# robin-karlsson0/pc-accumulation-lib

Measured on AMD Instinct MI355X. Metric: Mpoints/s projected+accumulated and BEV frames/s @256x256; 1/2/4/8 GPU, higher is better.
Workload: dtype f64; 1 GPU; KITTI-360 single forward cam, 120k pts/frame, 200 m horizon (~201 live frames, 5169634 stored pts), one 256x256x21 BEV per integrated frame; points_per_frame=120000, bev_px=256, view_m=80

## Files before the change

pc-accumulation-lib_amd/csrc/pca_bev.hip:

```cpp
#include "pca_bev_common.h"
#include "pca_k1_body.h"
#include <cstdlib>
#include <mutex>

#define KEY_INVALID 0xffffffffu
#define TS 8
#define TCELLS (TS * TS)
#define NFK (2 * TCELLS)
#ifndef AB_THREADS
#define AB_THREADS 1024
#endif
#define MAX_G 512
#ifndef BIN_RUNR
#define BIN_RUNR 4
#endif
#ifndef BIN_WPE
#define BIN_WPE 4
#endif
#ifndef BIN_UNR
#define BIN_UNR 4
#endif
#ifndef BIN_REG_P
#define BIN_REG_P 12
#endif
#ifndef C_THREADS
#define C_THREADS 256
#endif
#define C_WAVES (C_THREADS / 64)
#define C_HIST_WAVES 4
#define RGB_CAP 4096
#ifndef C_SLOT_Q
#define C_SLOT_Q 4
#endif
#define CONTIG_MIN 2560
#define HEAVY_MIN_DEFAULT 2560
#define FLAG_ROAD (1u << 24)
#define FLAG_DYNOBJ (1u << 25)

struct __attribute__((aligned(16))) RecF { double z; uint32_t iw; uint32_t cw; };
struct RecD { double z; double inten; uint32_t c; uint32_t fk; };

struct alignas(16) BevArgs {
    pca_store st;
    const double *intensity64;
    const int64_t *frame_off;
    int slot_begin, slot_split, slot_end;
    int64_t max_points;
    pca_bev_params prm;
    int n_pend;
    int write_back;
    int pend_slot_end[PCA_BEV_MAX_CHAIN];
    Mat34 pend_T[PCA_BEV_MAX_CHAIN];
    int tx, T, G;
    int Gr, Gp;
    int tile_mult;
    int heavy_min;
    int stagger;
    uint32_t *key;
    uint32_t *bh;
    uint32_t *boff;
    int Gk;
    int bin_first, bin_end;
    int k1_slot, k1_n;
    uint32_t *bh0;
    int split;
    uint32_t *heavy_hint;
    uint32_t heavy_hint_known;
    uint32_t *span_hint;
    uint32_t span_hint_known;
    int heavy_launched;
    uint32_t *heavy;
    void *recs;
    double *planes;
    uint16_t *planes_f16;
    double *extra;
    uint32_t *status;
    int dbg;
    int band_r0, band_rows;
};
#define HQ_CLASSES 32
#define HQ_CURSOR 32
#define HQ_DONE 33
#define HQ_IDS 64

struct Window { int64_t lo, hi, sp, c_lo, c_hi; };

__device__ __forceinline__ int chunk_index(const BevArgs &a, int64_t lo, int64_t sp, int64_t chunk)
{
    (void)a; (void)lo; (void)sp; (void)chunk;
    return (int)blockIdx.x;
}
#define K1_SEG 4096
#define K1_RIDE 32
__device__ __forceinline__ int64_t window_end(const BevArgs &a)
{
    const int e = a.Gk ? a.k1_slot : a.slot_end;
    return a.frame_off[a.bin_end < e ? a.bin_end : e];
}
__device__ __forceinline__ int64_t window_begin(const BevArgs &a) { return a.frame_off[a.bin_first]; }
__device__ __forceinline__ Window chunk_of(const BevArgs &a, int &g)
{
    Window w;
    w.lo = window_begin(a);
    const int64_t hi0 = window_end(a);
    w.sp = (a.Gk && a.slot_split > a.k1_slot) ? hi0 : a.frame_off[a.slot_split];
    w.hi = (hi0 - w.lo > a.max_points) ? w.lo + a.max_points : hi0;
    const int G = a.G - a.Gk;
    const int64_t chunk = (w.hi - w.lo + G - 1) / G;
    g = chunk_index(a, w.lo, w.sp, chunk);
    const int c = g - a.Gk;
    w.c_lo = w.lo + (int64_t)c * chunk;
    w.c_hi = w.c_lo + chunk < w.hi ? w.c_lo + chunk : w.hi;
    if (w.c_lo > w.hi) w.c_lo = w.c_hi = w.hi;
    return w;
}
__host__ __device__ __forceinline__ int64_t seg_stride(int64_t n, int G) { return (n + G - 1) / G; }
__device__ __forceinline__ bool bev_split(const BevArgs &a, int64_t window_points)
{
    return a.split == 2 || (a.split == 1 && window_points <= (int64_t)(a.G - a.Gk) * BIN_REG_P * AB_THREADS);
}
__device__ __forceinline__ int table_pos(const BevArgs &a, int g) { return a.Gp ? (g & 7) * a.Gp + (g >> 3) : g; }
__device__ __forceinline__ int table_group(const BevArgs &a, int p)
{
    if (!a.Gp) return p;
    const int x = p / a.Gp;
    return (p - x * a.Gp) * 8 + x;
}

struct BinPoint { double x, y, z; uint32_t key; };
struct PendHi { int64_t v[PCA_BEV_MAX_CHAIN]; };
__device__ __forceinline__ bool apply_owed(const BevArgs &a, const PendHi &pend_hi, int64_t p, double &X, double &Y, double &Z)
{
    bool moved = false;
#pragma unroll 1
    for (int k = 0; k < a.n_pend; ++k) {
        const int64_t hi = k == 0 ? pend_hi.v[0] : k == 1 ? pend_hi.v[1] : k == 2 ? pend_hi.v[2] : pend_hi.v[3];
        if (p < hi) {
            const Mat34 &T = a.pend_T[k];
            const double nx = row4(T.m + 0, X, Y, Z), ny = row4(T.m + 4, X, Y, Z), nz = row4(T.m + 8, X, Y, Z);
            X = nx; Y = ny; Z = nz;
            moved = true;
        }
    }
    return moved;
}
__device__ __forceinline__ uint32_t view_key(const BevArgs &a, const Window &w, int64_t p, double X, double Y, double Z, uint8_t D)
{
    const pca_bev_params &q = a.prm;
    const double v = q.view, vlo = -0.5 * v, vhi = 0.5 * v, pxd = (double)q.px, half_px = 0.5 * pxd;
    const bool use_h = !(q.height_filter != q.height_filter);
    const double x = X - q.origin[0];
    const double y = Y - q.origin[1];
    const double z = Z - q.origin[2];
    double ax = q.R[0] * x; ax = fma(q.R[1], y, ax); ax = fma(q.R[2], z, ax);
    double ay = q.R[3] * x; ay = fma(q.R[4], y, ay); ay = fma(q.R[5], z, ay);
    double az = q.R[6] * x; az = fma(q.R[7], y, az); az = fma(q.R[8], z, az);
    ax += q.dx;
    ay += q.dy;
    bool keep = (ax > vlo) && (ax < vhi) && (ay > vlo) && (ay < vhi);
    if (use_h) keep = keep && (az < q.height_filter);
    keep = keep && (D != 1);
    uint32_t key = KEY_INVALID;
    if (keep) {
        int i = (int)floor(ax / v * pxd + half_px);
        int j = (int)floor(ay / v * pxd + half_px);
        i = i > q.px - 1 ? q.px - 1 : (i < 0 ? 0 : i);
        j = j > q.px - 1 ? q.px - 1 : (j < 0 ? 0 : j);
        const int row = q.px - 1 - j, col = i;
        const uint32_t tile = (uint32_t)((row / TS) * a.tx + (col / TS));
        const uint32_t fk = (uint32_t)(((row % TS) * TS + (col % TS)) * 2) + (p >= w.sp ? 1u : 0u);
        key = (tile << 7) | fk;
    }
    return key;
}
struct ViewConst;
template <bool BAND = false>
__device__ __forceinline__ uint32_t view_key_lean(const ViewConst &c, double X, double Y, double Z, bool live, uint32_t set);
template <bool BAND>
__device__ __forceinline__ BinPoint bin_point(const BevArgs &a, const ViewConst &vc, const Window &w, const PendHi &pend_hi, int64_t p,
                                              double X, double Y, double Z, uint8_t D)
{
    BinPoint r;
    const bool moved = apply_owed(a, pend_hi, p, X, Y, Z);
    if (moved && a.write_back) { a.st.x[p] = X; a.st.y[p] = Y; a.st.z[p] = Z; }
    r.x = X; r.y = Y; r.z = Z;
    r.key = view_key_lean<BAND>(vc, X, Y, Z, D != 1, p >= w.sp ? 1u : 0u);
    return r;
}
template <bool I64>
__device__ __forceinline__ void bin_store(const BevArgs &a, const uint32_t *dynbits, uint32_t pos, uint32_t key, uint32_t rgbs, double z_store,
                                          double iv, float iv32)
{
    const pca_bev_params &q = a.prm;
    const unsigned sem = rgbs >> 24;
    uint32_t c = rgbs & 0xffffffu;
    if ((int)sem == q.road_class) c |= FLAG_ROAD;
    if ((dynbits[sem >> 5] >> (sem & 31u)) & 1u) c |= FLAG_DYNOBJ;
    const double z = z_store - q.origin[2];
    if (I64) {
        RecD r; r.z = z; r.inten = iv; r.c = c; r.fk = key & 127u;
        reinterpret_cast<RecD *>(a.recs)[pos] = r;
    } else {
        const float fi = iv32;
        if (fi < 0.0f) pca_raise(a.status, PCA_STATUS_NEGATIVE_INTENSITY);
        RecF r; r.z = z;
        r.iw = (__float_as_uint(fi) & 0x7fffffffu) | ((key & 1u) << 31);
        r.cw = c | (((key & 127u) >> 1) << 26);
        reinterpret_cast<RecF *>(a.recs)[pos] = r;
    }
}

struct ViewConst { double ox, oy, oz, r0, r1, r3, r4, dx, dy, vlo, vhi, v, rv, pxd, half_px, hf; int px, tx; bool use_h; uint32_t br0, brows; };
__device__ __forceinline__ ViewConst view_const(const BevArgs &a)
{
    const pca_bev_params &q = a.prm;
    ViewConst c;
    c.ox = q.origin[0]; c.oy = q.origin[1]; c.oz = q.origin[2];
    c.r0 = q.R[0]; c.r1 = q.R[1]; c.r3 = q.R[3]; c.r4 = q.R[4];
    c.dx = q.dx; c.dy = q.dy;
    c.v = q.view; c.rv = 1.0 / q.view; c.vlo = -0.5 * q.view; c.vhi = 0.5 * q.view; c.pxd = (double)q.px; c.half_px = 0.5 * c.pxd;
    c.hf = q.height_filter; c.use_h = !(q.height_filter != q.height_filter);
    c.px = q.px; c.tx = a.tx;
    c.br0 = (uint32_t)a.band_r0; c.brows = (uint32_t)a.band_rows;
    return c;
}
template <bool BAND>
__device__ __forceinline__ uint32_t view_key_lean(const ViewConst &c, double X, double Y, double Z, bool live, uint32_t set)
{
    const double x = X - c.ox, y = Y - c.oy;
    const double ax = fma(c.r1, y, c.r0 * x) + c.dx;
    const double ay = fma(c.r4, y, c.r3 * x) + c.dy;
    bool keep = live && (ax > c.vlo) && (ax < c.vhi) && (ay > c.vlo) && (ay < c.vhi) && (fabs(Z) < __builtin_huge_val());
    if (c.use_h) keep = keep && (Z - c.oz < c.hf);
    uint32_t key = KEY_INVALID;
    if (keep) {
// ... 583 lines not shown
}
__device__ __forceinline__ void hist16_add(uint32_t *row, unsigned val, uint32_t times)
{
    atomicAdd(&row[val >> 1], times << (16 * (val & 1)));
}
__device__ __forceinline__ void hist16_medians(TileStats &S, const uint32_t *row_p, const uint32_t *row_f, int cell, int ch,
                                               uint32_t n_p, uint32_t n_f)
{
    const uint4 p = hist16_bins(row_p), f = hist16_bins(row_f);
    const uint4 u = make_uint4(p.x + f.x, p.y + f.y, p.z + f.z, p.w + f.w);
    const uint32_t s_p = p.x + p.y + p.z + p.w, s_f = f.x + f.y + f.z + f.w;
    const uint32_t e_p = wave_incl_scan_add(s_p) - s_p, e_f = wave_incl_scan_add(s_f) - s_f;
    const uint32_t m_p = hist_med2_scanned(p, e_p, s_p, n_p), m_f = hist_med2_scanned(f, e_f, s_f, n_f),
                   m_u = hist_med2_scanned(u, e_p + e_f, s_p + s_f, n_p + n_f);
    if ((threadIdx.x & 63) == 0) { S.med2[0][cell][ch] = m_p; S.med2[1][cell][ch] = m_f; S.med2[2][cell][ch] = m_u; }
}

struct TileLds {
    TileStats S;
    uint32_t off[NFK + 1];
    uint32_t n_big;
    union {
        unsigned long long bits[TCELLS][24];
        uint32_t whist[C_HIST_WAVES][2][3][128];
        uint16_t owner[RGB_CAP];
    };
};

__device__ __forceinline__ void small_cells_bitplanes(TileLds &L, const uint32_t *s_rgb)
{
    const int lane = threadIdx.x & 63, wave = threadIdx.x >> 6;
    constexpr int PER_WAVE = TCELLS / C_WAVES;
    static_assert(PER_WAVE <= 64, "one lane per cell of the wave");
    uint32_t n_mine = 0;
    if (lane < PER_WAVE) n_mine = L.S.cnt[2 * (C_WAVES * lane + wave)] + L.S.cnt[2 * (C_WAVES * lane + wave) + 1];
    unsigned long long half = __ballot(n_mine >= 1 && n_mine <= 32), full = __ballot(n_mine > 32 && n_mine <= 64);
    while (half) {
        const int ia = __ffsll(half) - 1;
        half &= half - 1;
        const int ib = half ? __ffsll(half) - 1 : -1;
        half &= half - 1;
        const int i = lane < 32 ? ia : ib;
        const int l = lane & 31;
        uint32_t v = 0;
        int cell = 0;
        if (i >= 0) {
            cell = C_WAVES * i + wave;
            const uint32_t n = L.S.cnt[2 * cell] + L.S.cnt[2 * cell + 1];
            if ((uint32_t)l < n) v = s_rgb[L.off[2 * cell] + l];
        }
        const uint32_t t = wave_bit_transpose32(v);
        if (i >= 0 && l < 24) L.bits[cell][l] = (unsigned long long)t;
    }
    while (full) {
        const int i = __ffsll(full) - 1;
        full &= full - 1;
        const int cell = C_WAVES * i + wave;
        const uint32_t n = L.S.cnt[2 * cell] + L.S.cnt[2 * cell + 1];
        const uint32_t v = (uint32_t)lane < n ? s_rgb[L.off[2 * cell] + lane] : 0u;
        const uint32_t t = wave_bit_transpose32(v);
        if ((lane & 31) < 24) reinterpret_cast<uint32_t *>(&L.bits[cell][lane & 31])[lane >> 5] = t;
    }
}

template <typename W>
__device__ __forceinline__ uint32_t bitplane_select(const unsigned long long *planes, W cand, uint32_t k)
{
    uint32_t val = 0;
#pragma unroll
    for (int b = 7; b >= 0; --b) {
        const W B = (W)planes[b];
        const W zeros = cand & ~B;
        const uint32_t cz = sizeof(W) == 8 ? (uint32_t)__popcll((unsigned long long)zeros) : (uint32_t)__popc((uint32_t)zeros);
        const bool take0 = k < cz;
        cand = take0 ? zeros : (W)(cand & B);
        k = take0 ? k : k - cz;
        val |= take0 ? 0u : (1u << b);
    }
    return val;
}

__device__ __forceinline__ void small_cells_select(TileLds &L)
{
    const int lane = threadIdx.x & 63, wave = threadIdx.x >> 6;
    constexpr int NT = (TCELLS / C_WAVES) * 18;
    for (int t0 = 0; t0 < NT; t0 += 64) {
        const int t = t0 + lane;
        const int i = t / 18, qq = t - 18 * i;
        const int cell = C_WAVES * i + wave;
        const int set = qq / 6, ch = (qq % 6) >> 1, upper = qq & 1;
        bool ok = t < NT;
        uint32_t n_p = 0, n_f = 0;
        if (ok) { n_p = L.S.cnt[2 * cell]; n_f = L.S.cnt[2 * cell + 1]; }
        const uint32_t n = n_p + n_f;
        ok = ok && n > 0 && n <= 64;
        const unsigned long long m_p = n_p >= 64 ? ~0ull : ((1ull << n_p) - 1ull);
        const unsigned long long m_all = n >= 64 ? ~0ull : ((1ull << n) - 1ull);
        const unsigned long long cand = set == 0 ? m_p : (set == 1 ? (m_all & ~m_p) : m_all);
        const uint32_t n_s = (uint32_t)__popcll(cand);
        ok = ok && n_s > 0;
        const uint32_t k = upper ? (n_s >> 1) : ((n_s - 1) >> 1);
        uint32_t val = 0;
        const unsigned long long *planes = &L.bits[ok ? cell : 0][8 * ch];
        if (__any(ok && n > 32)) {
            if (ok) val = bitplane_select<unsigned long long>(planes, cand, k);
        } else {
            if (ok) val = bitplane_select<uint32_t>(planes, (uint32_t)cand, k);
        }
        const uint32_t other = dpp_or<0xb1>(0u, val);
        if (ok && !upper) L.S.med2[set][cell][ch] = val + other;
    }
}

__device__ __forceinline__ void wave_cells_hist(TileLds &L, const uint32_t *s_rgb)
{
    const int lane = threadIdx.x & 63, wave = threadIdx.x >> 6;
    if (wave >= C_HIST_WAVES) return;
    uint32_t *h = &L.whist[wave][0][0][0];
    for (int i = 0; i < TCELLS / C_HIST_WAVES; ++i) {
        const int cell = C_HIST_WAVES * i + wave;
        const uint32_t n_p = L.S.cnt[2 * cell], n_f = L.S.cnt[2 * cell + 1], n = n_p + n_f;
        if (n <= 64) continue;
        for (int k = lane; k < 2 * 3 * 128 / 4; k += 64) reinterpret_cast<uint4 *>(h)[k] = make_uint4(0, 0, 0, 0);
        const uint32_t base = L.off[2 * cell];
        for (uint32_t i0 = 0; i0 < n; i0 += 64) {
            const uint32_t idx = i0 + lane;
            const bool act = idx < n;
            const uint32_t v = act ? s_rgb[base + idx] : 0u;
            const uint32_t set = idx >= n_p ? 1u : 0u;
            const uint32_t tag = act ? (v | (set << 24)) : 0xffffffffu;
            const uint32_t first = __builtin_amdgcn_readfirstlane(tag);
            const uint64_t actm = __ballot(act);
            if (__ballot(tag == first) == actm && first != 0xffffffffu) {
                if (lane == (int)__ffsll((unsigned long long)actm) - 1) {
#pragma unroll
                    for (int ch = 0; ch < 3; ++ch)
                        hist16_add(&L.whist[wave][set][ch][0], (v >> (8 * ch)) & 255u, (uint32_t)__popcll(actm));
                }
            } else if (act) {
#pragma unroll
                for (int ch = 0; ch < 3; ++ch) hist16_add(&L.whist[wave][set][ch][0], (v >> (8 * ch)) & 255u, 1u);
            }
        }
#pragma unroll
        for (int ch = 0; ch < 3; ++ch) hist16_medians(L.S, &L.whist[wave][0][ch][0], &L.whist[wave][1][ch][0], cell, ch, n_p, n_f);
    }
}

template <bool I64, int NT>
__device__ __forceinline__ void tile_cell_medians32(TileStats &S, uint32_t (*hist)[256], const RecMap &M, const BevArgs &a, int cell,
                                                    uint32_t r_lo, uint32_t r_hi);

template <bool I64, bool BAND = false>
__device__ __forceinline__ void cells_drain(const BevArgs &a, TileLds &L, unsigned char *s_buf, bool pushed)
{
    TileStats &S = L.S;
    if (a.heavy_launched) return;
    __shared__ uint32_t s_drain_n;
    if (threadIdx.x == 0) {
        uint32_t n = 0;
        if (pushed) __threadfence();
        if (__hip_atomic_fetch_add(&a.heavy[HQ_DONE], 1u, __ATOMIC_RELAXED, __HIP_MEMORY_SCOPE_AGENT) == gridDim.x - 1) {
            __threadfence();
            for (int c = 0; c < HQ_CLASSES; ++c) n += __hip_atomic_load(&a.heavy[c], __ATOMIC_RELAXED, __HIP_MEMORY_SCOPE_AGENT);
            if (a.heavy_hint && n != a.heavy_hint_known) *a.heavy_hint = n;
        }
        s_drain_n = n;
    }
    __syncthreads();
    if (s_drain_n == 0) return;
    __threadfence();
    const bool extra = a.extra != nullptr;
    const bool div255 = !I64 && a.prm.intensity_div255;
    RecMap &M = *reinterpret_cast<RecMap *>(s_buf);
    uint32_t (*hist)[256] = reinterpret_cast<uint32_t (*)[256]>(s_buf + ((sizeof(RecMap) + 15) & ~(size_t)15));
    static_assert(((sizeof(RecMap) + 15) & ~(size_t)15) + 3 * 256 * 4 <= RGB_CAP * 4, "RecMap + histograms live in the colour buffer");
    for (int cls = 0; cls < HQ_CLASSES; ++cls) {
        const uint32_t n_cls = __hip_atomic_load(&a.heavy[cls], __ATOMIC_RELAXED, __HIP_MEMORY_SCOPE_AGENT);
        for (uint32_t k = 0; k < n_cls; ++k) {
            const int tile = (int)__hip_atomic_load(&a.heavy[HQ_IDS + (size_t)cls * a.T + k], __ATOMIC_RELAXED, __HIP_MEMORY_SCOPE_AGENT);
            __syncthreads();
            stats_init(S, C_THREADS);
            const uint32_t r_hi = recmap_build(M, a, tile, C_THREADS);
            Run run;
            run_reset(run, RUN_NONE);
            const uint32_t per_thread = (r_hi + C_THREADS - 1) / C_THREADS;
            const uint32_t t_lo = threadIdx.x * per_thread, t_hi = t_lo + per_thread < r_hi ? t_lo + per_thread : r_hi;
            for (uint32_t r = t_lo; r < t_hi; ++r) {
                uint32_t kk, c;
                double z, iv;
                load_rec<I64>(a, recmap_at(M, a.Gr, r), kk, c, z, iv);
                if (kk != run.key) {
                    if (run.key != RUN_NONE) run_flush(S, extra, run);
                    run_reset(run, kk);
                }
                run_add(run, extra, c, z, iv, div255);
            }
            if (run.key != RUN_NONE) run_flush(S, extra, run);
            __syncthreads();
            uint32_t *h16 = &L.whist[0][0][0][0];
            for (int c0 = 0; c0 < TCELLS; c0 += 4) {
                uint32_t any = 0;
                for (int c = c0; c < c0 + 4; ++c) any += S.cnt[2 * c] + S.cnt[2 * c + 1];
                if (any == 0) continue;
                for (int k = threadIdx.x; k < 8 * 3 * 128 / 4; k += C_THREADS) reinterpret_cast<uint4 *>(h16)[k] = make_uint4(0, 0, 0, 0);
                __syncthreads();
                for (uint32_t r = threadIdx.x; r < r_hi; r += C_THREADS) {
                    uint32_t kk, v;
                    load_rec_key_colour<I64>(a, recmap_at(M, a.Gr, r), kk, v);
                    const uint32_t rel = kk - 2u * (uint32_t)c0;
                    if (rel >= 8u) continue;
#pragma unroll
                    for (int ch = 0; ch < 3; ++ch) hist16_add(h16 + (rel * 3 + ch) * 128, (v >> (8 * ch)) & 255u, 1u);
                }
                __syncthreads();
                const int wave = threadIdx.x >> 6;
                for (int job = wave; job < 4 * 3; job += C_THREADS / 64) {
                    const int cl = job / 3, ch = job % 3, cell = c0 + cl;
                    const uint32_t n_p = S.cnt[2 * cell], n_f = S.cnt[2 * cell + 1];
                    if (n_p + n_f == 0 || n_p > 0xffffu || n_f > 0xffffu) continue;
                    hist16_medians(S, h16 + ((2 * cl) * 3 + ch) * 128, h16 + ((2 * cl + 1) * 3 + ch) * 128, cell, ch, n_p, n_f);
                }
                __syncthreads();
                for (int cell = c0; cell < c0 + 4; ++cell)
                    if (S.cnt[2 * cell] > 0xffffu || S.cnt[2 * cell + 1] > 0xffffu)
                        tile_cell_medians32<I64, C_THREADS>(S, hist, M, a, cell, 0u, r_hi);
            }
            __syncthreads();
            tile_finalize_write<BAND>(a, S, reinterpret_cast<double(*)[TCELLS]>(s_buf), tile, C_THREADS);
        }
    }
}

#define DBG_STAMP(bit, slot) do { if ((a.dbg & (bit)) && threadIdx.x == 0 && tile < 1024) g_dbg_stamps[tile][slot] = wall_clock64(); } while (0)
template <bool I64, bool BAND = false>
__device__ __forceinline__ void bev_tile_cells_body(const BevArgs &a)
{
    __shared__ TileLds L;
    __shared__ __align__(16) unsigned char s_buf[RGB_CAP * 4 > OUT_STAGE_BYTES ? RGB_CAP * 4 : OUT_STAGE_BYTES];
    uint32_t *s_rgb = reinterpret_cast<uint32_t *>(s_buf);
    const int lane = threadIdx.x & 63, wave = threadIdx.x >> 6;
    const bool extra = a.extra != nullptr;
    int tile;
    if (!BAND && (a.tx & 3) == 0) {
        const int Tq = a.T >> 2, bw = a.tx >> 2;
        const int q = (int)blockIdx.x / Tq, i = (int)blockIdx.x - q * Tq;
        const int i2 = (int)(((int64_t)i * a.tile_mult) % Tq);
        const int row = q * bw + i2 / a.tx, col = (i2 % a.tx + q * bw) % a.tx;
        tile = row * a.tx + col;
    } else {
        tile = (int)(((int64_t)blockIdx.x * a.tile_mult) % a.T);
    }
    if (a.stagger > 0) {
        const int slot = (int)blockIdx.x / ((a.T + 3) >> 2);
        for (int k = 0; k < slot * a.stagger; ++k) __builtin_amdgcn_s_sleep(16);
    }
    const unsigned long long t_begin = wall_clock64();
    RecMap &M = *reinterpret_cast<RecMap *>(s_buf);
    static_assert(sizeof(RecMap) <= sizeof(s_buf), "RecMap aliases the colour buffer");
    stats_init(L.S, C_THREADS);
    const uint32_t r_lo = 0, r_hi = recmap_build(M, a, tile, C_THREADS, L.owner);
    if (r_hi > (uint32_t)a.heavy_min) {
        if (threadIdx.x == 0) heavy_push(a, tile, r_hi);
        cells_drain<I64, BAND>(a, L, s_buf, true);
        return;
    }

    constexpr int RPT = RGB_CAP / C_THREADS;
    constexpr int HALF = RPT / 2;
    constexpr int Q = C_SLOT_Q;
    static_assert(RPT % Q == 0, "whole rounds");
    const bool contig = (r_hi - r_lo) > CONTIG_MIN;
    const bool div255 = !I64 && a.prm.intensity_div255;
    const uint32_t n_slots = contig ? (uint32_t)RPT : __builtin_amdgcn_readfirstlane((r_hi - r_lo + C_THREADS - 1) / C_THREADS);
    uint32_t kr[RPT], cc[RPT];
    auto load_round = [&](auto rec, auto &k, auto &c, auto &z, auto &iv) {
        constexpr int N = sizeof(k) / sizeof(k[0]);
        if constexpr (I64) {
#pragma unroll
            for (int u = 0; u < N; ++u) {
                const uint32_t r = rec(u);
                k[u] = RUN_NONE; c[u] = 0; z[u] = 0; iv[u] = 0;
                if (r < r_hi) load_rec<I64>(a, recmap_at(M, L.owner, r), k[u], c[u], z[u], iv[u]);
            }
        } else {
            uint4 w[N];
#pragma unroll
            for (int u = 0; u < N; ++u) {
                const uint32_t r = rec(u);
                w[u] = recf_raw(a, recmap_at(M, L.owner, r < r_hi ? r : r_lo));
            }
#pragma unroll
            for (int u = 0; u < N; ++u) {
                recf_fields(w[u], k[u], c[u], z[u], iv[u]);
                if (!(rec(u) < r_hi)) { k[u] = RUN_NONE; c[u] = 0; }
            }
        }
    };
    if (r_hi == r_lo) {
#pragma unroll
        for (int uu = 0; uu < RPT; ++uu) { kr[uu] = RUN_NONE; cc[uu] = 0; }
    } else if (!contig) {
#pragma unroll
        for (int uu = 0; uu < RPT; ++uu) { kr[uu] = RUN_NONE; cc[uu] = 0; }
#pragma unroll
        for (int h = 0; h < RPT / Q; ++h) {
            if ((uint32_t)(h * Q) >= n_slots) continue;
            uint32_t k[Q], c[Q];
            double z[Q], iv[Q];
            load_round([&](int u) { return r_lo + (uint32_t)(h * Q + u) * C_THREADS + threadIdx.x; }, k, c, z, iv);
#pragma unroll
            for (int u = 0; u < Q; ++u) {
                const int uu = h * Q + u;
                cc[uu] = c[u] & 0xffffffu;
                if (k[u] != RUN_NONE) kr[uu] = k[u] | (rec_add(L.S, extra, k[u], c[u], z[u], iv[u], div255) << 8);
            }
        }
    } else {
        uint32_t end_base[RPT];
        uint32_t is_end = 0;
        Run run;
        run_reset(run, RUN_NONE);
#pragma unroll
        for (int h = 0; h < 2; ++h) {
            uint32_t k[HALF], c[HALF];
            double z[HALF], iv[HALF];
            load_round([&](int u) { return r_lo + threadIdx.x * RPT + (uint32_t)(h * HALF + u); }, k, c, z, iv);
#pragma unroll
            for (int u = 0; u < HALF; ++u) {
                const int uu = h * HALF + u;
                kr[uu] = RUN_NONE; cc[uu] = c[u] & 0xffffffu; end_base[uu] = 0;
                if (k[u] == RUN_NONE) continue;
                if (k[u] != run.key) {
                    if (run.key != RUN_NONE && uu > 0) { end_base[uu - 1] = run_flush(L.S, extra, run); is_end |= 1u << (uu - 1); }
                    run_reset(run, k[u]);
                }
                kr[uu] = k[u] | (run.cnt << 8);
                run_add(run, extra, c[u], z[u], iv[u], div255);
            }
        }
        uint32_t b = run.key != RUN_NONE ? run_flush(L.S, extra, run) : 0u;
#pragma unroll
        for (int uu = RPT - 1; uu >= 0; --uu) {
            if ((is_end >> uu) & 1u) b = end_base[uu];
            if (kr[uu] != RUN_NONE) kr[uu] += b << 8;
        }
    }
    __syncthreads();
    DBG_STAMP(16, 3);
    if (wave == 0) {
        const uint32_t c0 = L.S.cnt[2 * lane], c1 = L.S.cnt[2 * lane + 1];
        const uint32_t inc = wave_incl_scan_add(c0 + c1);
        const uint32_t excl = inc - (c0 + c1);
        L.off[2 * lane] = excl;
        L.off[2 * lane + 1] = excl + c0;
        if (lane == 63) L.off[NFK] = inc;
        const unsigned long long big = __ballot(c0 + c1 > 64);
        if (lane == 0) L.n_big = (uint32_t)__popcll(big);
    }
    __syncthreads();
#pragma unroll
    for (int h = 0; h < RPT / Q; ++h) {
        if ((uint32_t)(h * Q) >= n_slots) continue;
#pragma unroll
        for (int u = h * Q; u < (h + 1) * Q; ++u)
            if (kr[u] != 0xffffffffu) s_rgb[L.off[kr[u] & 127u] + (kr[u] >> 8)] = cc[u];
    }
    __syncthreads();
    DBG_STAMP(16, 4);
    small_cells_bitplanes(L, s_rgb);
    __syncthreads();
    small_cells_select(L);
    __syncthreads();
    DBG_STAMP(16, 5);
    if (L.n_big) {
        wave_cells_hist(L, s_rgb);
        __syncthreads();
    }
    DBG_STAMP(16, 6);
    tile_finalize_write<BAND>(a, L.S, reinterpret_cast<double(*)[TCELLS]>(s_buf), tile, C_THREADS);
    cells_drain<I64, BAND>(a, L, s_buf, false);
    if ((a.dbg & 16) && threadIdx.x == 0 && tile < 1024) {
        g_dbg_stamps[tile][0] = t_begin; g_dbg_stamps[tile][1] = wall_clock64(); g_dbg_stamps[tile][2] = r_hi - r_lo;
        uint32_t big = 0;
        for (int c = 0; c < TCELLS; ++c) big += (L.S.cnt[2 * c] + L.S.cnt[2 * c + 1]) > 64;
        g_dbg_stamps[tile][7] = __smid() | ((unsigned long long)big << 32);
    }
}

#define H_THREADS 1024
#define H_CELLS 32
#define H_HIST_DWORDS (H_CELLS * 2 * 3 * 128)
struct HeavyLds {
    TileStats S;
    RecMap M;
    uint32_t hist[3][256];
    uint32_t overflow;
};
#define HEAVY_LDS_BYTES (H_HIST_DWORDS * 4 + sizeof(HeavyLds))

template <bool I64, int NT>
__device__ __forceinline__ void tile_hist32(uint32_t (*hist)[256], const RecMap &M, const BevArgs &a, uint32_t fk, uint32_t r_lo,
                                            uint32_t r_hi)
{
    const int lane = threadIdx.x & 63;
    for (uint32_t r0 = r_lo; r0 < r_hi; r0 += NT) {
        const uint32_t r = r0 + threadIdx.x;
        bool act = r < r_hi;
        uint32_t v = 0;
        if (act) {
            uint32_t k;
            load_rec_key_colour<I64>(a, recmap_at(M, a.Gr, r), k, v);
            act = k == fk;
        }
        const uint32_t tag = act ? v : 0xffffffffu;
        const uint32_t first = __builtin_amdgcn_readfirstlane(tag);
        const uint64_t actm = __ballot(act);
        if (actm == 0) continue;
        if (__ballot(tag == first) == actm && first != 0xffffffffu) {
            if (lane == (int)__ffsll((unsigned long long)actm) - 1) {
#pragma unroll
                for (int ch = 0; ch < 3; ++ch) atomicAdd(&hist[ch][(v >> (8 * ch)) & 255u], (uint32_t)__popcll(actm));
            }
        } else if (act) {
#pragma unroll
            for (int ch = 0; ch < 3; ++ch) atomicAdd(&hist[ch][(v >> (8 * ch)) & 255u], 1u);
        }
    }
}
template <bool I64, int NT>
__device__ __forceinline__ void tile_cell_medians32(TileStats &S, uint32_t (*hist)[256], const RecMap &M, const BevArgs &a, int cell,
                                                    uint32_t r_lo, uint32_t r_hi)
{
    const int lane = threadIdx.x & 63, wave = threadIdx.x >> 6;
    const uint32_t n_p = S.cnt[2 * cell], n_f = S.cnt[2 * cell + 1];
    for (int round = 0; round < 2; ++round) {
        for (int i = threadIdx.x; i < 3 * 256; i += NT) (&hist[0][0])[i] = 0;
        __syncthreads();
        if (round == 0) {
            tile_hist32<I64, NT>(hist, M, a, 2 * cell, r_lo, r_hi);
            __syncthreads();
            if (wave < 3) { const uint32_t m = hist_med2(hist[wave], n_p); if (lane == 0) S.med2[0][cell][wave] = m; }
            __syncthreads();
        }
        tile_hist32<I64, NT>(hist, M, a, 2 * cell + 1, r_lo, r_hi);
        __syncthreads();
        if (wave < 3) {
            const uint32_t m = hist_med2(hist[wave], round == 0 ? n_p + n_f : n_f);
            if (lane == 0) S.med2[round == 0 ? 2 : 1][cell][wave] = m;
        }
        __syncthreads();
    }
}

template <bool I64, bool EXTRA, bool OWN, bool BAND = false>
__device__ __forceinline__ void bev_tile_cells_heavy_body(const BevArgs &a)
{
    unsigned long long t_begin = wall_clock64();
    extern __shared__ __align__(16) unsigned char smem[];
    uint32_t *hist = reinterpret_cast<uint32_t *>(smem);
    HeavyLds &L = *reinterpret_cast<HeavyLds *>(smem + (size_t)H_HIST_DWORDS * 4);
    __shared__ uint32_t s_next;
    const int wave = threadIdx.x >> 6, lane = threadIdx.x & 63;
    constexpr bool extra = EXTRA;
    const bool div255 = !I64 && a.prm.intensity_div255;
    __shared__ uint32_t s_cls[HQ_CLASSES + 1];
    if (threadIdx.x == 0) {
        uint32_t run = 0;
        for (int c = 0; c < HQ_CLASSES; ++c) { s_cls[c] = run; run += a.heavy[c]; }
        s_cls[HQ_CLASSES] = run;
    }
    __syncthreads();
    const uint32_t n_heavy = s_cls[HQ_CLASSES];
    if (a.heavy_hint && blockIdx.x == 0 && threadIdx.x == 0 && n_heavy != a.heavy_hint_known) *a.heavy_hint = n_heavy;
    constexpr int HALVES = TCELLS / H_CELLS;
    for (;;) {
    if (threadIdx.x == 0) s_next = atomicAdd(&a.heavy[HQ_CURSOR], 1u);
    __syncthreads();
    const uint32_t item = s_next;
    if (item >= n_heavy * HALVES) break;
    int tile;
    {
        const uint32_t ti = item / HALVES;
        int cls = 0;
        while (cls + 1 < HQ_CLASSES && s_cls[cls + 1] <= ti) ++cls;
        tile = (int)a.heavy[HQ_IDS + (size_t)cls * a.T + (ti - s_cls[cls])];
    }
    const int half = (int)(item % HALVES);
    if (item >= (uint32_t)gridDim.x) t_begin = wall_clock64();
    stats_init(L.S, H_THREADS);
    bool own = false;
    if (OWN) {
        const int64_t wn = window_end(a) - window_begin(a);
        own = bev_split(a, wn > a.max_points ? a.max_points : wn);
    }
    const uint32_t r_lo = 0, r_hi = recmap_build(L.M, a, tile, H_THREADS, nullptr, OWN ? half : -1);
    if (threadIdx.x == 0) L.overflow = 0;
    {
        for (int k = threadIdx.x; k < H_HIST_DWORDS / 4; k += H_THREADS) reinterpret_cast<uint4 *>(hist)[k] = make_uint4(0, 0, 0, 0);
        __syncthreads();
        constexpr int UNR = 4;
        Run run;
        run_reset(run, RUN_NONE);
        for (uint32_t r0 = r_lo + threadIdx.x * UNR; r0 < r_hi; r0 += H_THREADS * UNR) {
            uint32_t k[UNR], c[UNR];
            double z[UNR], iv[UNR];
            RecWalk walk;
            recwalk_seek(walk, L.M, a.Gr, r0);
            if constexpr (I64) {
#pragma unroll
                for (int u = 0; u < UNR; ++u) {
                    k[u] = RUN_NONE; c[u] = 0; z[u] = 0; iv[u] = 0;
                    if (r0 + u < r_hi) load_rec<I64>(a, recwalk_next(walk, L.M, a.Gr, r_hi), k[u], c[u], z[u], iv[u]);
                }
            } else {
                uint32_t at[UNR];
                uint4 w[UNR];
                const uint32_t at0 = walk.at;
#pragma unroll
                for (int u = 0; u < UNR; ++u) at[u] = r0 + u < r_hi ? recwalk_next(walk, L.M, a.Gr, r_hi) : at0;
#pragma unroll
                for (int u = 0; u < UNR; ++u) w[u] = recf_raw(a, at[u]);
#pragma unroll
                for (int u = 0; u < UNR; ++u) {
                    recf_fields(w[u], k[u], c[u], z[u], iv[u]);
                    if (!(r0 + u < r_hi)) { k[u] = RUN_NONE; c[u] = 0; }
                }
            }
#pragma unroll
            for (int u = 0; u < UNR; ++u) {
                if (k[u] == RUN_NONE || (!own && (int)(k[u] >> 1) / H_CELLS != half)) continue;
                if (k[u] != run.key) {
                    if (run.key != RUN_NONE) run_flush(L.S, extra, run);
                    run_reset(run, k[u]);
// ... 563 lines not shown
```

Baseline: 1457 Mpoints/s.

## Process heavy tiles in their own block instead of a last-block drain queue

Before, a block that found a heavy tile pushed it to a global queue, and the last block to finish (found through an atomic done counter) serially processed every queued heavy tile. Now, when no separate heavy kernel is launched, the block that owns the heavy tile processes it directly, and the done counter and the drain call at the end of every block are removed. This spreads heavy-tile work across many blocks in parallel and drops one global atomic plus fences per block. The heavy hint is now set to 1 rather than to the real count, which may change how the host sizes or launches the heavy path on later calls.

After: 1554 Mpoints/s, median of 6. 6.6% higher.

```diff
diff --git a/pc-accumulation-lib_amd/csrc/pca_bev.hip b/pc-accumulation-lib_amd/csrc/pca_bev.hip
--- a/pc-accumulation-lib_amd/csrc/pca_bev.hip
+++ b/pc-accumulation-lib_amd/csrc/pca_bev.hip
@@ -80,7 +80,6 @@
 };
 #define HQ_CLASSES 32
 #define HQ_CURSOR 32
-#define HQ_DONE 33
 #define HQ_IDS 64
 
 struct Window { int64_t lo, hi, sp, c_lo, c_hi; };
@@ -970,84 +969,64 @@
                                                     uint32_t r_lo, uint32_t r_hi);
 
 template <bool I64, bool BAND = false>
-__device__ __forceinline__ void cells_drain(const BevArgs &a, TileLds &L, unsigned char *s_buf, bool pushed)
+__device__ __forceinline__ void cells_heavy_here(const BevArgs &a, TileLds &L, unsigned char *s_buf, int tile)
 {
     TileStats &S = L.S;
-    if (a.heavy_launched) return;
-    __shared__ uint32_t s_drain_n;
-    if (threadIdx.x == 0) {
-        uint32_t n = 0;
-        if (pushed) __threadfence();
-        if (__hip_atomic_fetch_add(&a.heavy[HQ_DONE], 1u, __ATOMIC_RELAXED, __HIP_MEMORY_SCOPE_AGENT) == gridDim.x - 1) {
-            __threadfence();
-            for (int c = 0; c < HQ_CLASSES; ++c) n += __hip_atomic_load(&a.heavy[c], __ATOMIC_RELAXED, __HIP_MEMORY_SCOPE_AGENT);
-            if (a.heavy_hint && n != a.heavy_hint_known) *a.heavy_hint = n;
-        }
-        s_drain_n = n;
-    }
-    __syncthreads();
-    if (s_drain_n == 0) return;
-    __threadfence();
+    if (threadIdx.x == 0 && a.heavy_hint && a.heavy_hint_known == 0) *a.heavy_hint = 1u;
     const bool extra = a.extra != nullptr;
     const bool div255 = !I64 && a.prm.intensity_div255;
     RecMap &M = *reinterpret_cast<RecMap *>(s_buf);
     uint32_t (*hist)[256] = reinterpret_cast<uint32_t (*)[256]>(s_buf + ((sizeof(RecMap) + 15) & ~(size_t)15));
     static_assert(((sizeof(RecMap) + 15) & ~(size_t)15) + 3 * 256 * 4 <= RGB_CAP * 4, "RecMap + histograms live in the colour buffer");
-    for (int cls = 0; cls < HQ_CLASSES; ++cls) {
-        const uint32_t n_cls = __hip_atomic_load(&a.heavy[cls], __ATOMIC_RELAXED, __HIP_MEMORY_SCOPE_AGENT);
-        for (uint32_t k = 0; k < n_cls; ++k) {
-            const int tile = (int)__hip_atomic_load(&a.heavy[HQ_IDS + (size_t)cls * a.T + k], __ATOMIC_RELAXED, __HIP_MEMORY_SCOPE_AGENT);
-            __syncthreads();
-            stats_init(S, C_THREADS);
-            const uint32_t r_hi = recmap_build(M, a, tile, C_THREADS);
-            Run run;
-            run_reset(run, RUN_NONE);
-            const uint32_t per_thread = (r_hi + C_THREADS - 1) / C_THREADS;
-            const uint32_t t_lo = threadIdx.x * per_thread, t_hi = t_lo + per_thread < r_hi ? t_lo + per_thread : r_hi;
-            for (uint32_t r = t_lo; r < t_hi; ++r) {
-                uint32_t kk, c;
-                double z, iv;
-                load_rec<I64>(a, recmap_at(M, a.Gr, r), kk, c, z, iv);
-                if (kk != run.key) {
-                    if (run.key != RUN_NONE) run_flush(S, extra, run);
-                    run_reset(run, kk);
-                }
-                run_add(run, extra, c, z, iv, div255);
-            }
+    __syncthreads();
+    stats_init(S, C_THREADS);
+    const uint32_t r_hi = recmap_build(M, a, tile, C_THREADS);
+    Run run;
+    run_reset(run, RUN_NONE);
+    const uint32_t per_thread = (r_hi + C_THREADS - 1) / C_THREADS;
+    const uint32_t t_lo = threadIdx.x * per_thread, t_hi = t_lo + per_thread < r_hi ? t_lo + per_thread : r_hi;
+    for (uint32_t r = t_lo; r < t_hi; ++r) {
+        uint32_t kk, c;
+        double z, iv;
+        load_rec<I64>(a, recmap_at(M, a.Gr, r), kk, c, z, iv);
+        if (kk != run.key) {
             if (run.key != RUN_NONE) run_flush(S, extra, run);
-            __syncthreads();
-            uint32_t *h16 = &L.whist[0][0][0][0];
-            for (int c0 = 0; c0 < TCELLS; c0 += 4) {
-                uint32_t any = 0;
-                for (int c = c0; c < c0 + 4; ++c) any += S.cnt[2 * c] + S.cnt[2 * c + 1];
-                if (any == 0) continue;
-                for (int k = threadIdx.x; k < 8 * 3 * 128 / 4; k += C_THREADS) reinterpret_cast<uint4 *>(h16)[k] = make_uint4(0, 0, 0, 0);
-                __syncthreads();
-                for (uint32_t r = threadIdx.x; r < r_hi; r += C_THREADS) {
-                    uint32_t kk, v;
-                    load_rec_key_colour<I64>(a, recmap_at(M, a.Gr, r), kk, v);
-                    const uint32_t rel = kk - 2u * (uint32_t)c0;
-                    if (rel >= 8u) continue;
-#pragma unroll
-                    for (int ch = 0; ch < 3; ++ch) hist16_add(h16 + (rel * 3 + ch) * 128, (v >> (8 * ch)) & 255u, 1u);
-                }
-                __syncthreads();
-                const int wave = threadIdx.x >> 6;
-                for (int job = wave; job < 4 * 3; job += C_THREADS / 64) {
-                    const int cl = job / 3, ch = job % 3, cell = c0 + cl;
-                    const uint32_t n_p = S.cnt[2 * cell], n_f = S.cnt[2 * cell + 1];
-                    if (n_p + n_f == 0 || n_p > 0xffffu || n_f > 0xffffu) continue;
-                    hist16_medians(S, h16 + ((2 * cl) * 3 + ch) * 128, h16 + ((2 * cl + 1) * 3 + ch) * 128, cell, ch, n_p, n_f);
-                }
-                __syncthreads();
-                for (int cell = c0; cell < c0 + 4; ++cell)
-                    if (S.cnt[2 * cell] > 0xffffu || S.cnt[2 * cell + 1] > 0xffffu)
-                        tile_cell_medians32<I64, C_THREADS>(S, hist, M, a, cell, 0u, r_hi);
-            }
-            __syncthreads();
-            tile_finalize_write<BAND>(a, S, reinterpret_cast<double(*)[TCELLS]>(s_buf), tile, C_THREADS);
-        }
-    }
+            run_reset(run, kk);
+        }
+        run_add(run, extra, c, z, iv, div255);
+    }
+    if (run.key != RUN_NONE) run_flush(S, extra, run);
+    __syncthreads();
+    uint32_t *h16 = &L.whist[0][0][0][0];
+    for (int c0 = 0; c0 < TCELLS; c0 += 4) {
+        uint32_t any = 0;
+        for (int c = c0; c < c0 + 4; ++c) any += S.cnt[2 * c] + S.cnt[2 * c + 1];
+        if (any == 0) continue;
+        for (int k = threadIdx.x; k < 8 * 3 * 128 / 4; k += C_THREADS) reinterpret_cast<uint4 *>(h16)[k] = make_uint4(0, 0, 0, 0);
+        __syncthreads();
+        for (uint32_t r = threadIdx.x; r < r_hi; r += C_THREADS) {
+            uint32_t kk, v;
+            load_rec_key_colour<I64>(a, recmap_at(M, a.Gr, r), kk, v);
+            const uint32_t rel = kk - 2u * (uint32_t)c0;
+            if (rel >= 8u) continue;
+#pragma unroll
+            for (int ch = 0; ch < 3; ++ch) hist16_add(h16 + (rel * 3 + ch) * 128, (v >> (8 * ch)) & 255u, 1u);
+        }
+        __syncthreads();
+        const int wave = threadIdx.x >> 6;
+        for (int job = wave; job < 4 * 3; job += C_THREADS / 64) {
+            const int cl = job / 3, ch = job % 3, cell = c0 + cl;
+            const uint32_t n_p = S.cnt[2 * cell], n_f = S.cnt[2 * cell + 1];
+            if (n_p + n_f == 0 || n_p > 0xffffu || n_f > 0xffffu) continue;
+            hist16_medians(S, h16 + ((2 * cl) * 3 + ch) * 128, h16 + ((2 * cl + 1) * 3 + ch) * 128, cell, ch, n_p, n_f);
+        }
+        __syncthreads();
+        for (int cell = c0; cell < c0 + 4; ++cell)
+            if (S.cnt[2 * cell] > 0xffffu || S.cnt[2 * cell + 1] > 0xffffu)
+                tile_cell_medians32<I64, C_THREADS>(S, hist, M, a, cell, 0u, r_hi);
+    }
+    __syncthreads();
+    tile_finalize_write<BAND>(a, S, reinterpret_cast<double(*)[TCELLS]>(s_buf), tile, C_THREADS);
 }
 
 #define DBG_STAMP(bit, slot) do { if ((a.dbg & (bit)) && threadIdx.x == 0 && tile < 1024) g_dbg_stamps[tile][slot] = wall_clock64(); } while (0)
@@ -1079,8 +1058,8 @@
     stats_init(L.S, C_THREADS);
     const uint32_t r_lo = 0, r_hi = recmap_build(M, a, tile, C_THREADS, L.owner);
     if (r_hi > (uint32_t)a.heavy_min) {
-        if (threadIdx.x == 0) heavy_push(a, tile, r_hi);
-        cells_drain<I64, BAND>(a, L, s_buf, true);
+        if (a.heavy_launched) { if (threadIdx.x == 0) heavy_push(a, tile, r_hi); }
+        else cells_heavy_here<I64, BAND>(a, L, s_buf, tile);
         return;
     }
 
@@ -1197,7 +1176,6 @@
     }
     DBG_STAMP(16, 6);
     tile_finalize_write<BAND>(a, L.S, reinterpret_cast<double(*)[TCELLS]>(s_buf), tile, C_THREADS);
-    cells_drain<I64, BAND>(a, L, s_buf, false);
     if ((a.dbg & 16) && threadIdx.x == 0 && tile < 1024) {
         g_dbg_stamps[tile][0] = t_begin; g_dbg_stamps[tile][1] = wall_clock64(); g_dbg_stamps[tile][2] = r_hi - r_lo;
         uint32_t big = 0;
```
